# stdstu12/YUME

Hardware: NVIDIA H100
Metric: latent_frames_per_sec (higher is better)
Workload: dtype bf16

## Files before the change

### include/yume_b200.h

```cpp
#ifndef YUME_B200_H_
#define YUME_B200_H_

#ifdef __cplusplus
extern "C" {
#endif

#define YB_OK 0
#define YB_ERR_ARG (-1)
#define YB_ERR_SHAPE (-2)
#define YB_ERR_ALIGNMENT (-3)
#define YB_ERR_NO_DRIVER (-4)
#define YB_ERR_TENSORMAP (-5)
#define YB_ERR_LAUNCH (-6)

int yb_abi_version(void);

#define YB_EPI_BF16 0
#define YB_EPI_GELU_BF16 1
#define YB_EPI_F32 2
#define YB_EPI_GATE_RES 3
#define YB_EPI_RES_BF16 5
#define YB_EPI_GELU_ERF_BF16 4

typedef struct yb_gemm_args {
// ... 3 lines not shown
  const void* B;
  const void* bias;
  void* out;
  const void* gate;
  const void* tok_idx;
  long long lda, ldb, ldo, gate_ld;
  int M, N, K;
  int epilogue;
  int block_n;
  int n_split;
  long long split_stride;
  int a_split;
  long long a_split_stride;
  const void* res;
  long long res_ld;
  int split_k;
  void* ws;
  long long ws_bytes;
} yb_gemm_args;
int yb_gemm_bf16(const yb_gemm_args* args, void* stream);
long long yb_gemm_workspace_bytes(int M, int N, int K, int epilogue, int cta_pair, int split_k);
int yb_gemm_splitk_plan(int tiles, int num_kb, int clusters, int split_k, int* out3);
int yb_gemm_plan(int M, int N, int sms, int* out4);

typedef struct yb_conv3d_args {
  unsigned int struct_bytes;
  int cta_pair;
  const void* xpad;
  const void* w;
  const void* bias;
  void* out;
  const void* res;
  long long ldo, res_ld;
  int T, H, W, Cp, Cout;
  int epilogue;
  int kt, kh, kw;
  int oob_zero_pad;
  int out_t_mul, out_t_add;
  int fuse_w;
  int stride_t, stride_hw;
} yb_conv3d_args;
int yb_conv3d_causal(const yb_conv3d_args* args, void* stream);
int yb_conv3d_plan(int T, int H, int W, int Cout, int kw, int fuse_w, int* out4);

int yb_ln_modulate(const void* x, long long ldx, void* out, long long ldo, int out_f32, const void* scale,
                   const void* shift, long long mod_ld, const void* tok_idx, const void* weight, const void* lnbias,
// ... 77 lines not shown
```

### yume_b200/_lib.py

```python
from __future__ import annotations

import ctypes as C
from pathlib import Path

_LIB_PATH = Path(__file__).resolve().parent / "csrc" / "libyume_b200.so"

YB_EPI_BF16, YB_EPI_GELU_BF16, YB_EPI_F32, YB_EPI_GATE_RES, YB_EPI_GELU_ERF_BF16, YB_EPI_RES_BF16 = 0, 1, 2, 3, 4, 5
YB_ATT_P_SMEM, YB_ATT_ACCUMULATE = 1, 2
ABI_VERSION = 4
YB_ATT_EMU_SHIFT, YB_ATT_SPLIT_SHIFT = 2, 4

_ERRORS = {
    -1: "YB_ERR_ARG (null pointer / bad enum / non-positive size)",
    -2: "YB_ERR_SHAPE (shape not supported by the kernel)",
    -3: "YB_ERR_ALIGNMENT (pointer or stride not 16-byte aligned)",
    -4: "YB_ERR_NO_DRIVER (cuTensorMapEncodeTiled unavailable: no CUDA driver)",
    -5: "YB_ERR_TENSORMAP (driver rejected a TMA descriptor)",
    -6: "YB_ERR_LAUNCH (kernel launch failed)",
}


class YumeB200Error(RuntimeError):
    pass

# ... 15 lines not shown
class Conv3dArgs(C.Structure):

    _fields_ = [
        ("struct_bytes", C.c_uint), ("cta_pair", C.c_int),
        ("xpad", C.c_void_p), ("w", C.c_void_p), ("bias", C.c_void_p), ("out", C.c_void_p), ("res", C.c_void_p),
        ("ldo", C.c_longlong), ("res_ld", C.c_longlong),
        ("T", C.c_int), ("H", C.c_int), ("W", C.c_int), ("Cp", C.c_int), ("Cout", C.c_int), ("epilogue", C.c_int),
        ("kt", C.c_int), ("kh", C.c_int), ("kw", C.c_int), ("oob_zero_pad", C.c_int), ("out_t_mul", C.c_int),
        ("out_t_add", C.c_int), ("fuse_w", C.c_int), ("stride_t", C.c_int), ("stride_hw", C.c_int),
    ]


_vp, _ll, _i, _f = C.c_void_p, C.c_longlong, C.c_int, C.c_float
SIGNATURES = {
    "yb_abi_version": (_i, []),
    "yb_gemm_bf16": (_i, [C.POINTER(GemmArgs), _vp]),
    "yb_conv3d_causal": (_i, [C.POINTER(Conv3dArgs), _vp]),
    "yb_gn_stats": (_i, [_vp, _ll, _vp, _ll, _i, _i, _vp]),
    "yb_vae_pad_act": (_i, [_vp, _ll, _i, _i, _i, _i, _vp, _i, _i, _i, _i, _i, _vp, _vp, _vp, _i, _f, _i, _vp]),
    "yb_masked_softmax": (_i, [_vp, _ll, _vp, _ll, _i, _i, _vp]),
    "yb_nchw_to_nhwc_bf16": (_i, [_vp, _vp, _ll, _i, _i, _vp]),
    "yb_nhwc_to_nchw_f32": (_i, [_vp, _ll, _vp, _ll, _i, _vp]),
    "yb_gemm_plan": (_i, [_i, _i, _i, C.POINTER(C.c_int)]),
    "yb_gemm_workspace_bytes": (_ll, [_i, _i, _i, _i, _i, _i]),
    "yb_gemm_splitk_plan": (_i, [_i, _i, _i, _i, C.POINTER(C.c_int)]),
    "yb_conv3d_plan": (_i, [_i, _i, _i, _i, _i, _i, C.POINTER(C.c_int)]),
    "yb_attention_plan": (_i, [_i, _i, _i, _i, _i, C.POINTER(C.c_int)]),
    "yb_nhwc_to_nchw_f32_clamp": (_i, [_vp, _ll, _vp, _ll, _i, C.c_float, C.c_float, _vp]),
    "yb_blend": (_i, [_vp, _vp, _ll, _i, _i, _i, _ll, _vp]),
    "yb_vae_assemble_tiles": (_i, [_vp, _vp, _vp, _vp, _vp, _i, _i, _i, _i, _i, _i, _i, _i, _i, _i, _i, _vp, _vp]),
    "yb_vae_rms_act": (_i, [_vp, _ll, _vp, _vp, _i, _i, _i, _i, _i, _i, _i, _vp]),
    "yb_vae_dupup_add": (_i, [_vp, _vp, _i, _i, _i, _i, _i, _i, _i, _vp]),
    "yb_vae_unpatchify2_clamp": (_i, [_vp, _ll, _vp, _i, _i, _i, _vp]),
    "yb_vae_avgdown_add": (_i, [_vp, _vp, _i, _i, _i, _i, _i, _i, _i, _vp]),
    "yb_vae_patchify2_bf16": (_i, [_vp, _vp, _ll, _i, _i, _i, _vp]),
    "yb_ln_modulate": (_i, [_vp, _ll, _vp, _ll, _i, _vp, _vp, _ll, _vp, _vp, _vp, _i, _i, _f, _vp]),
    "yb_rmsnorm_rope": (_i, [_vp, _ll, _vp, _vp, _i, _i, _i, _i, _f, _vp]),
    "yb_rmsnorm_rope_pieces": (_i, [_vp, _ll, _i, _ll, _vp, _vp, _i, _i, _i, _i, _f, _vp]),
    "yb_qk_norm_rope": (_i, [_vp, _vp, _ll, _i, _ll, _vp, _vp, _vp, _i, _i, _i, _i, _f, _vp]),
    "yb_attention": (_i, [_vp, _ll, _vp, _ll, _vp, _ll, _vp, _ll, _i, _i, _i, _f, _i, _vp]),
    "yb_attention_ex": (_i, [_vp, _ll, _vp, _ll, _vp, _ll, _vp, _ll, _i, _i, _i, _f, _i, _vp, _ll, _vp, _vp]),
    "yb_attention_workspace_bytes": (_ll, [_i, _i, _i, _i, _i]),
    "yb_debug_force_split": (_i, [_i]),
    "yb_sp_scatter_qkv": (_i, [_vp, _ll, _vp, _vp, _vp, _i, _i, _i, _i, _f, C.POINTER(C.c_void_p), _i, _i, _i, _vp]),
    "yb_gemm_sp_qkv": (_i, [_vp, _ll, _vp, _vp, _i, _i, _i, C.POINTER(C.c_void_p), _i, _i, _i, _vp, _vp]),
    "yb_sp_bcast_sums": (_i, [_vp, C.POINTER(C.c_void_p), _i, _i, _i, _vp]),
# ... 107 lines not shown
```

### yume_b200/csrc/gemm.cu

```cuda
#include "yb_host.h"
#include "../../include/yume_b200_stream.h"
#include "yb_ptx.cuh"

namespace yb {

constexpr int GEMM_BLOCK_M = 128;
constexpr int GEMM_BLOCK_K = 64;
constexpr int GEMM_THREADS = 384;
constexpr int GEMM_MAX_STAGES = 8;
constexpr int GEMM_SMEM_BYTES = 227 * 1024;
constexpr int GEMM_A_BYTES = GEMM_BLOCK_M * GEMM_BLOCK_K * 2;
constexpr int GEMM_EPI_STAGE_BYTES = 8 * 16 * 36 * 4;
constexpr int GEMM_EPI_BOX_BYTES = 64 * 128;
constexpr int GEMM_EPI_TMA_BYTES = 2 * 2 * GEMM_EPI_BOX_BYTES;

struct GemmParams {
  int M, N, K;
  const float* bias;
  void* out;
  long long ldo;
  const float* gate;
  long long gate_ld;
  const int* tok_idx;
  int a_split;
// ... 6 lines not shown
  int cT, cH, cW;
  int kh, kw;
  int off_t, off_h, off_w;
  int out_t_mul, out_t_add;
  int st_t, st_h, st_w;
  int num_m_tiles, num_n_tiles;
  int block_n, stages;
  int sk_full, sk_ns, sk_per;
  float* sk_ws;
  int tma_out;
  __nv_bfloat16* sp_peers[8];
  float* sp_sums;
  int sp_rank, sp_Lp, sp_Wh, sp_C;
};
constexpr int YB_EPI_SP_QKV = 6;

constexpr int CONVW_ROWS = GEMM_BLOCK_M + 2;
constexpr int CONVW_A_SLAB = 17 * 1024;
constexpr int CONVW_A_STAGES = 4;

__host__ __device__ constexpr int gemm_b_bytes(int block_n) { return ((block_n + 63) / 64) * 64 * GEMM_BLOCK_K * 2; }
__host__ __device__ constexpr int gemm_stage_bytes(int block_n, int convw) { return (convw ? 0 : GEMM_A_BYTES) + gemm_b_bytes(block_n); }
__host__ __device__ constexpr int gemm_a_ring_bytes(int convw) { return convw ? CONVW_A_STAGES * CONVW_A_SLAB : 0; }
__host__ __device__ constexpr bool gemm_has_tma_epilogue(int epi, int convw, int cluster) {
  return cluster == 1 && !convw && (epi == YB_EPI_BF16 || epi == YB_EPI_GELU_BF16 || epi == YB_EPI_GELU_ERF_BF16 ||
                                    epi == YB_EPI_F32 || epi == YB_EPI_GATE_RES);
}
__host__ __device__ constexpr bool gemm_tma_epilogue_only(int epi, int convw, int cluster) {
  return gemm_has_tma_epilogue(epi, convw, cluster) && epi != YB_EPI_BF16 && epi != YB_EPI_F32;
}
__host__ __device__ constexpr int gemm_epi_bytes(bool tma) { return tma ? GEMM_EPI_TMA_BYTES : GEMM_EPI_STAGE_BYTES; }
static int gemm_stages(int block_n, int convw, int epi_bytes) {
  const int s = (GEMM_SMEM_BYTES - 1024 - 256 - epi_bytes - gemm_a_ring_bytes(convw)) / gemm_stage_bytes(block_n, convw);
  return s > GEMM_MAX_STAGES ? GEMM_MAX_STAGES : s;
}

template <int EPI>
__device__ __forceinline__ void epilogue_rows16(const GemmParams& p, int col0, int my_row, int my_tok, const float* stage, int lane,
                                                float* sq) {
  constexpr bool kBf16Out = (EPI == YB_EPI_BF16 || EPI == YB_EPI_GELU_BF16 || EPI == YB_EPI_GELU_ERF_BF16 ||
                             EPI == YB_EPI_RES_BF16 || EPI == YB_EPI_SP_QKV);
  if (col0 >= p.N) return;
  if (kBf16Out) {
    const int cq = (lane & 3) * 8;
    float b[8] = {0.f, 0.f, 0.f, 0.f, 0.f, 0.f, 0.f, 0.f};
    if (p.bias) {
      const float4 b0 = __ldg(reinterpret_cast<const float4*>(p.bias + col0 + cq));
      const float4 b1 = __ldg(reinterpret_cast<const float4*>(p.bias + col0 + cq + 4));
      b[0] = b0.x; b[1] = b0.y; b[2] = b0.z; b[3] = b0.w; b[4] = b1.x; b[5] = b1.y; b[6] = b1.z; b[7] = b1.w;
    }
    long long col_off = col0 + cq;
    if (p.n_split > 0) col_off = static_cast<long long>(col0 / p.n_split) * p.split_stride + (col0 % p.n_split) + cq;
// ... 170 lines not shown
}

template <int NM>
__device__ __forceinline__ void gemm_mma_k64(float (&acc)[128], uint32_t sa, uint32_t sb, int block_n, bool zero_first) {
  const uint64_t ad0 = make_smem_desc_sw128(sa, 16, 1024), bd0 = make_smem_desc_sw128(sb, 16, 1024);
  const int nb64 = (block_n + 63) >> 6;
#pragma unroll
  for (int k = 0; k < GEMM_BLOCK_K / 16; ++k) {
    const uint64_t ad = ad0 + 2 * k, bd = bd0 + 2 * k;
    const uint32_t accum = (zero_first && k == 0) ? 0u : 1u;
    if (NM == 256) {
      wgmma_ss_n256<0>(acc, ad, bd, accum);
    } else if (NM == 128) {
      wgmma_ss_n128<0>(acc, ad, bd, accum);
    } else {
      wgmma_ss_n64<0>(acc, ad, bd, accum);
      if (nb64 > 1) wgmma_ss_n64<32>(acc, ad, bd + (8192 >> 4), accum);
      if (nb64 > 2) wgmma_ss_n64<64>(acc, ad, bd + (16384 >> 4), accum);
      if (nb64 > 3) wgmma_ss_n64<96>(acc, ad, bd + (24576 >> 4), accum);
    }
  }
}

template <int CLUSTER>
__device__ __forceinline__ void release_slot(uint64_t* bar, int lane) {
  __syncwarp();
  if (lane == 0) {
    if (CLUSTER == 1) {
      mbar_arrive(bar);
    } else {
      mbar_arrive_cluster(bar, 0);
      mbar_arrive_cluster(bar, 1);
    }
  }
}

template <int EPI, int CONVW, int CLUSTER, int NM>
__global__ void __launch_bounds__(GEMM_THREADS, 1)
gemm_kernel(const __grid_constant__ CUtensorMap tmA, const __grid_constant__ CUtensorMap tmB, const __grid_constant__ CUtensorMap tmO,
            const GemmParams p) {
  static_assert(!(CONVW && CLUSTER != 1), "the kw-fused conv runs on single CTAs");
  constexpr bool kTmaEpi = gemm_has_tma_epilogue(EPI, CONVW, CLUSTER);
  const bool tma_out = gemm_tma_epilogue_only(EPI, CONVW, CLUSTER) || (kTmaEpi && p.tma_out);
  extern __shared__ uint8_t smem_raw[];
  uint8_t* smem = reinterpret_cast<uint8_t*>((reinterpret_cast<uintptr_t>(smem_raw) + 1023) & ~uintptr_t(1023));
  const int block_n = p.block_n, stages = p.stages;
  const int stage_bytes = gemm_stage_bytes(block_n, CONVW);
  uint8_t* a_ring = smem + stages * stage_bytes;
  float* epi = reinterpret_cast<float*>(a_ring + gemm_a_ring_bytes(CONVW));
  uint64_t* full_bar = reinterpret_cast<uint64_t*>(reinterpret_cast<uint8_t*>(epi) + gemm_epi_bytes(kTmaEpi));
  uint64_t* empty_bar = full_bar + GEMM_MAX_STAGES;
  uint64_t* a_full = empty_bar + GEMM_MAX_STAGES;
  uint64_t* a_empty = a_full + CONVW_A_STAGES;

  const int warp = threadIdx.x >> 5, lane = threadIdx.x & 31;
  const int rank = CLUSTER == 2 ? static_cast<int>(cluster_ctarank()) : 0;
  const int tile_first = blockIdx.x / CLUSTER, tile_step = gridDim.x / CLUSTER;
  const int num_tiles = p.num_m_tiles * p.num_n_tiles;
  const int num_kb = (p.K + GEMM_BLOCK_K - 1) / GEMM_BLOCK_K;
  const int num_work = p.sk_full + (num_tiles - p.sk_full) * p.sk_ns;
  auto decode_work = [&](int w, int& tile, int& kb0, int& kb1, int& part) {
    tile = w; kb0 = 0; kb1 = num_kb; part = -1;
    if (w >= p.sk_full) {
      const int u = w - p.sk_full;
      tile = p.sk_full + u / p.sk_ns;
      kb0 = (u % p.sk_ns) * p.sk_per;
      kb1 = min(num_kb, kb0 + p.sk_per);
      part = u;
    }
  };
  auto conv_box = [&](int mt, int& it, int& ih, int& iw) {
    const int per_t = p.tiles_h * p.tiles_w;
    it = mt / per_t;
    const int rem = mt - it * per_t;
    ih = rem / p.tiles_w;
    iw = rem - ih * p.tiles_w;
  };

  if (threadIdx.x == 0) {
    tma_prefetch_desc(&tmA);
    tma_prefetch_desc(&tmB);
    if (tma_out) tma_prefetch_desc(&tmO);
    for (int i = 0; i < stages; ++i) {
      mbar_init(&full_bar[i], 1);
      mbar_init(&empty_bar[i], 8 * CLUSTER);
    }
    for (int i = 0; i < (CONVW ? CONVW_A_STAGES : 0); ++i) {
      mbar_init(&a_full[i], 1);
      mbar_init(&a_empty[i], 8);
    }
    fence_barrier_init();
  }
  __syncthreads();
  if (CLUSTER > 1) cluster_sync_all();

  if (warp < 4) {
    setmaxnreg_dec<40>();
    if (warp == 0 && lane == 0) {
      int stage = 0, a_stage = 0;
      uint32_t phase = 0, a_phase = 0;
      for (int w = tile_first; w < num_work; w += tile_step) {
        int tile, kb0, kb1, part, m_tile, n_tile;
        decode_work(w, tile, kb0, kb1, part);
        tile_coords(tile, p.num_m_tiles, p.num_n_tiles, m_tile, n_tile);
        if (CONVW) {
          int it, ih, iw;
          conv_box(m_tile, it, ih, iw);
          const int groups = num_kb / 3;
// ... 3 lines not shown
            mbar_wait(&a_empty[a_stage], a_phase ^ 1);
            mbar_arrive_expect_tx(&a_full[a_stage], CONVW_ROWS * GEMM_BLOCK_K * 2);
            tma_load_4d(a_ring + a_stage * CONVW_A_SLAB, &tmA, &a_full[a_stage], cc * GEMM_BLOCK_K, iw * GEMM_BLOCK_M - p.off_w,
                        ih + dh - p.off_h, it + dt - p.off_t);
            if (++a_stage == CONVW_A_STAGES) {
              a_stage = 0;
              a_phase ^= 1;
            }
#pragma unroll 1
            for (int dw = 0; dw < 3; ++dw) {
              mbar_wait(&empty_bar[stage], phase ^ 1);
              mbar_arrive_expect_tx(&full_bar[stage], block_n * GEMM_BLOCK_K * 2);
              tma_load_2d(smem + stage * stage_bytes, &tmB, &full_bar[stage], ((tdh * 3 + dw) * p.cin_chunks + cc) * GEMM_BLOCK_K,
                          n_tile * block_n);
              if (++stage == stages) {
                stage = 0;
                phase ^= 1;
              }
            }
          }
          continue;
        }
        for (int kb = kb0; kb < kb1; ++kb) {
          if (CLUSTER > 1) mbar_wait_cluster(&empty_bar[stage], phase ^ 1);
          else mbar_wait(&empty_bar[stage], phase ^ 1);
          uint8_t* sa = smem + stage * stage_bytes;
          uint8_t* sb = sa + GEMM_A_BYTES;
          mbar_arrive_expect_tx(&full_bar[stage], GEMM_A_BYTES + block_n * GEMM_BLOCK_K * 2);
          const int kcol = kb * GEMM_BLOCK_K;
          const int mt = m_tile * CLUSTER + rank;
          if (p.conv) {
            const int tap = kb / p.cin_chunks, cc = kb - tap * p.cin_chunks;
            const int dt = tap / (p.kh * p.kw), dh = (tap / p.kw) % p.kh, dw = tap % p.kw;
            int it, ih, iw;
            conv_box(mt, it, ih, iw);
            tma_load_4d(sa, &tmA, &full_bar[stage], cc * GEMM_BLOCK_K, iw * p.TW * p.st_w + dw - p.off_w,
                        ih * p.TH * p.st_h + dh - p.off_h, it * p.TT * p.st_t + dt - p.off_t);
          } else {
            const int chunk = kcol / p.a_split;
            tma_load_3d(sa, &tmA, &full_bar[stage], kcol - chunk * p.a_split, mt * GEMM_BLOCK_M, chunk);
          }
          if (CLUSTER == 1) {
            tma_load_2d(sb, &tmB, &full_bar[stage], kcol, n_tile * block_n);
          } else {
            const int half = block_n / 2;
            tma_load_2d_multicast(sb + rank * half * GEMM_BLOCK_K * 2, &tmB, &full_bar[stage], kcol, n_tile * block_n + rank * half,
                                  static_cast<uint16_t>(3));
          }
          if (++stage == stages) {
            stage = 0;
            phase ^= 1;
          }
        }
      }
    }
  } else {
    setmaxnreg_inc<232>();
    const int wg = (warp >> 2) - 1;
    const int r0 = wg * 64 + (warp & 3) * 16;
    float* stage_buf = epi + (warp - 4) * (16 * 36);
    uint8_t* box_bufs = reinterpret_cast<uint8_t*>(epi) + wg * 2 * GEMM_EPI_BOX_BYTES;
    uint32_t nbox = 0;
    int stage = 0, a_stage = 0;
    uint32_t phase = 0, a_phase = 0;
    float acc[128];
// ... 20 lines not shown
      }
      if (EPI == YB_EPI_GATE_RES && part < 0 && my_row >= 0 && lane < 16) {
        const char* xrow = reinterpret_cast<const char*>(reinterpret_cast<const float*>(p.out) +
                                                         static_cast<long long>(my_row) * p.ldo + n_tile * block_n);
        const int ncols = min(block_n, p.N - n_tile * block_n);
        for (int b = 0; b < ncols * 4; b += 128) asm volatile("prefetch.global.L2 [%0];" ::"l"(xrow + b));
      }
      int prev = -1;
      if (CONVW) {
        int prev_a = -1;
        const int groups = num_kb / 3;
        for (int g = 0; g < groups; ++g) {
          mbar_wait(&a_full[a_stage], a_phase);
          const uint32_t sa = smem_u32(a_ring + a_stage * CONVW_A_SLAB) + wg * 64 * 128;
#pragma unroll 1
          for (int dw = 0; dw < 3; ++dw) {
            mbar_wait(&full_bar[stage], phase);
            fence_regs(acc);
            wgmma_fence();
            gemm_mma_k64<NM>(acc, sa + dw * 128, smem_u32(smem + stage * stage_bytes), block_n, g == 0 && dw == 0);
            wgmma_commit();
            wgmma_wait<1>();
            fence_regs(acc);
            if (prev >= 0) release_slot<1>(&empty_bar[prev], lane);
            if (dw == 0 && prev_a >= 0) {
              release_slot<1>(&a_empty[prev_a], lane);
              prev_a = -1;
            }
            prev = stage;
            if (++stage == stages) {
              stage = 0;
              phase ^= 1;
            }
          }
          prev_a = a_stage;
          if (++a_stage == CONVW_A_STAGES) {
            a_stage = 0;
            a_phase ^= 1;
          }
        }
        wgmma_wait<0>();
        fence_regs(acc);
        if (prev >= 0) release_slot<1>(&empty_bar[prev], lane);
        if (prev_a >= 0) release_slot<1>(&a_empty[prev_a], lane);
      } else {
        for (int kb = kb0; kb < kb1; ++kb) {
          mbar_wait(&full_bar[stage], phase);
          const uint32_t sa = smem_u32(smem + stage * stage_bytes);
          fence_regs(acc);
          wgmma_fence();
          gemm_mma_k64<NM>(acc, sa + wg * 64 * 128, sa + GEMM_A_BYTES, block_n, kb == kb0);
          wgmma_commit();
          wgmma_wait<1>();
          fence_regs(acc);
          if (prev >= 0) release_slot<CLUSTER>(&empty_bar[prev], lane);
          prev = stage;
          if (++stage == stages) {
            stage = 0;
            phase ^= 1;
          }
        }
        wgmma_wait<0>();
        fence_regs(acc);
        if (prev >= 0) release_slot<CLUSTER>(&empty_bar[prev], lane);
      }

      const int q4 = lane >> 2, c2 = 2 * (lane & 3);
      if (part >= 0) {
        float* wbase = p.sk_ws + (static_cast<long long>(part) * 256 + rank * GEMM_BLOCK_M + r0) * block_n;
#pragma unroll
        for (int g = 0; g < 32; ++g) {
          if (g * 8 < block_n) {
            *reinterpret_cast<float2*>(wbase + q4 * block_n + g * 8 + c2) = make_float2(acc[4 * g], acc[4 * g + 1]);
            *reinterpret_cast<float2*>(wbase + (q4 + 8) * block_n + g * 8 + c2) = make_float2(acc[4 * g + 2], acc[4 * g + 3]);
          }
        }
        continue;
      }
      if (tma_out) {
        epilogue_tma<EPI, NM>(p, &tmO, acc, box_bufs, mt * GEMM_BLOCK_M + wg * 64, n_tile * block_n, wg, threadIdx.x & 127, nbox);
        continue;
      }
      int my_tok = 0;
      if (EPI == YB_EPI_GATE_RES && p.gate != nullptr && p.tok_idx != nullptr && my_row >= 0) my_tok = p.tok_idx[my_row];
      float sq[2] = {0.f, 0.f};
      auto flush_sq = [&](int part_) {
#pragma unroll
// ... 101 lines not shown
}

template <typename Kern>
static int pair_max_clusters(Kern kern) {
  cudaLaunchConfig_t cfg = {};
  cfg.gridDim = dim3(2 * (sm_count() / 2));
  cfg.blockDim = dim3(GEMM_THREADS);
  cfg.dynamicSmemBytes = GEMM_SMEM_BYTES;
  cudaLaunchAttribute attr;
  attr.id = cudaLaunchAttributeClusterDimension;
  attr.val.clusterDim.x = 2;
  attr.val.clusterDim.y = 1;
  attr.val.clusterDim.z = 1;
  cfg.attrs = &attr;
  cfg.numAttrs = 1;
  int n = 0;
  if (cudaOccupancyMaxActiveClusters(&n, kern, &cfg) != cudaSuccess || n <= 0) {
    (void)cudaGetLastError();
    n = sm_count() / 2;
  }
  return n;
}

template <int EPI, int CONVW, int CLUSTER>
static int launch_gemm(const CUtensorMap& tmA, const CUtensorMap& tmB, const CUtensorMap* tmO, GemmParams& p, cudaStream_t stream,
                       int split_k = 1, void* ws = nullptr, long long ws_bytes = 0) {
  static const CUtensorMap no_map = {};
  if (gemm_tma_epilogue_only(EPI, CONVW, CLUSTER) && tmO == nullptr) return YB_ERR_ARG;
  p.tma_out = gemm_has_tma_epilogue(EPI, CONVW, CLUSTER) && tmO != nullptr;
  if (!p.tma_out) tmO = &no_map;
  const int nm = p.block_n == 256 ? 2 : p.block_n == 128 ? 1 : 0;
  if (CLUSTER == 1 && nm == 0) return YB_ERR_ARG;
  auto kern = nm == 2 ? gemm_kernel<EPI, CONVW, CLUSTER, 256> : nm == 1 ? gemm_kernel<EPI, CONVW, CLUSTER, 128>
                      : gemm_kernel<EPI, CONVW, CLUSTER, CLUSTER == 1 ? 128 : 64>;
  static bool attr_set[3][kMaxDevices] = {};
  if (int rc = ensure_dynamic_smem(kern, GEMM_SMEM_BYTES, attr_set[nm], "gemm")) return rc;
  if (CLUSTER == 2) p.num_m_tiles = p.conv ? (p.num_m_tiles + 1) / 2 : (p.M + 255) / 256;
  else if (!p.conv) p.num_m_tiles = (p.M + GEMM_BLOCK_M - 1) / GEMM_BLOCK_M;
  p.num_n_tiles = (p.N + p.block_n - 1) / p.block_n;
  p.stages = gemm_stages(p.block_n, CONVW, gemm_epi_bytes(gemm_has_tma_epilogue(EPI, CONVW, CLUSTER)));
  const int tiles = p.num_m_tiles * p.num_n_tiles;
  static int max_clusters[kMaxDevices] = {0};
  const int dev = current_device();
  if (max_clusters[dev] == 0) max_clusters[dev] = CLUSTER == 2 ? pair_max_clusters(kern) : sm_count();
  p.sk_full = tiles; p.sk_ns = 1; p.sk_per = 0; p.sk_ws = nullptr;
  int tail = 0;
  if (CLUSTER == 2 && EPI == YB_EPI_GATE_RES && !p.conv && ws != nullptr && split_k != 1) {
    const int num_kb = (p.K + GEMM_BLOCK_K - 1) / GEMM_BLOCK_K;
    gemm_splitk_plan(tiles, num_kb, max_clusters[dev], split_k, &p.sk_full, &p.sk_ns, &p.sk_per);
    tail = tiles - p.sk_full;
    const long long need = static_cast<long long>(tail) * p.sk_ns * 256 * p.block_n * 4;
    if (tail > 0 && (ws_bytes < need || (reinterpret_cast<uintptr_t>(ws) & 0xF))) {
      p.sk_full = tiles; p.sk_ns = 1; tail = 0;
    }
    if (tail > 0) p.sk_ws = static_cast<float*>(ws);
  }
  const int work = p.sk_full + tail * p.sk_ns;
  const int groups = work < max_clusters[dev] ? work : max_clusters[dev];
  cudaLaunchConfig_t cfg = {};
  cfg.gridDim = dim3(groups * CLUSTER);
  cfg.blockDim = dim3(GEMM_THREADS);
  cfg.dynamicSmemBytes = GEMM_SMEM_BYTES;
  cfg.stream = stream;
// ... 85 lines not shown
  if (tiles <= 0 || num_kb <= 0 || clusters <= 0 || split_k < 0 || split_k > 12 || !out3) return YB_ERR_ARG;
  yb::gemm_splitk_plan(tiles, num_kb, clusters, split_k, &out3[0], &out3[1], &out3[2]);
  return YB_OK;
}

extern "C" long long yb_gemm_workspace_bytes(int M, int N, int K, int epilogue, int cta_pair, int split_k) {
  using namespace yb;
  if (M <= 0 || N <= 0 || K <= 0 || epilogue != YB_EPI_GATE_RES || split_k == 1 || split_k < 0 || split_k > 12) return 0;
  if (cta_pair != 2) return 0;
  static int max_clusters[kMaxDevices] = {0};
  static bool attr_set[kMaxDevices] = {false};
  const int dev = current_device();
  if (max_clusters[dev] == 0) {
    if (ensure_dynamic_smem(gemm_kernel<YB_EPI_GATE_RES, 0, 2, 256>, GEMM_SMEM_BYTES, attr_set, "gemm")) return 0;
    max_clusters[dev] = pair_max_clusters(gemm_kernel<YB_EPI_GATE_RES, 0, 2, 256>);
  }
  const int bn = pair_block_n(M, N, max_clusters[dev]);
  const int tiles = ((M + 255) / 256) * ((N + bn - 1) / bn);
  int full, ns, per;
  gemm_splitk_plan(tiles, (K + GEMM_BLOCK_K - 1) / GEMM_BLOCK_K, max_clusters[dev], split_k, &full, &ns, &per);
  return static_cast<long long>(tiles - full) * ns * 256 * bn * 4;
}

extern "C" int yb_gemm_bf16(const yb_gemm_args* a, void* stream_) {
  using namespace yb;
  if (!a || !a->A || !a->B || !a->out) return YB_ERR_ARG;
  if (a->M <= 0 || a->N <= 0 || a->K <= 0) return YB_ERR_ARG;
  if (a->N % 32 != 0 || a->K % 8 != 0) return YB_ERR_SHAPE;
  if (a->epilogue < 0 || a->epilogue > YB_EPI_RES_BF16) return YB_ERR_ARG;
  if (a->epilogue == YB_EPI_RES_BF16 && (!a->res || (a->res_ld % 8))) return YB_ERR_ARG;
  if ((a->lda % 8) || (a->ldb % 8) || (a->ldo % 8) || (reinterpret_cast<uintptr_t>(a->out) & 0xF)) return YB_ERR_ALIGNMENT;
  cudaStream_t stream = reinterpret_cast<cudaStream_t>(stream_);
  if (a->struct_bytes != sizeof(yb_gemm_args)) return YB_ERR_ARG;
  if (a->cta_pair < 0 || a->cta_pair > 2 || a->split_k < 0 || a->split_k > 12) return YB_ERR_ARG;
  int a_split = a->K;
  long long a_chunk_ld = 0;
  if (a->a_split > 0) {
    if (a->a_split % GEMM_BLOCK_K != 0 || a->K % a->a_split != 0) return YB_ERR_SHAPE;
    a_split = a->a_split;
    a_chunk_ld = a->a_split_stride;
  }
  const int a_chunks = a->K / a_split;
  if (a->n_split < 0 || (a->n_split > 0 && (a->n_split % 32 != 0 || a->epilogue != YB_EPI_BF16))) return YB_ERR_ARG;
  GemmParams p;
  p.M = a->M;
  p.N = a->N;
  p.K = a->K;
  p.bias = static_cast<const float*>(a->bias);
  p.out = a->out;
  p.ldo = a->ldo;
  p.gate = static_cast<const float*>(a->gate);
  p.gate_ld = a->gate_ld;
  p.tok_idx = static_cast<const int*>(a->tok_idx);
  p.a_split = a_split;
  p.res = static_cast<const __nv_bfloat16*>(a->res);
  p.res_ld = a->res_ld;
  p.conv = 0;
// ... 3 lines not shown
  p.stages = 0;
  CUtensorMap tmA, tmB;
  int rc = make_tmap_bf16_3d(&tmA, a->A, a_chunks, a->M, a_split, a->lda, a_chunks > 1 ? a_chunk_ld : a->lda * (long long)a->M + 8,
                             GEMM_BLOCK_M, GEMM_BLOCK_K);
  if (rc) return rc;
  const bool pair = a->cta_pair == 2;
  if (pair) {
    int bn = a->block_n;
    if (bn == 0) bn = pair_block_n(a->M, a->N, sm_count() / 2);
    if (bn < 32 || bn > 256 || bn % 32 != 0) return YB_ERR_ARG;
    p.block_n = bn;
    rc = make_tmap_bf16_2d(&tmB, a->B, a->N, a->K, a->ldb, bn / 2, GEMM_BLOCK_K);
    if (rc) return rc;
    switch (a->epilogue) {
      case YB_EPI_BF16: return launch_gemm<YB_EPI_BF16, 0, 2>(tmA, tmB, nullptr, p, stream);
      case YB_EPI_GELU_BF16: return launch_gemm<YB_EPI_GELU_BF16, 0, 2>(tmA, tmB, nullptr, p, stream);
      case YB_EPI_F32: return launch_gemm<YB_EPI_F32, 0, 2>(tmA, tmB, nullptr, p, stream);
      case YB_EPI_GELU_ERF_BF16: return launch_gemm<YB_EPI_GELU_ERF_BF16, 0, 2>(tmA, tmB, nullptr, p, stream);
      case YB_EPI_RES_BF16: return launch_gemm<YB_EPI_RES_BF16, 0, 2>(tmA, tmB, nullptr, p, stream);
      default: return launch_gemm<YB_EPI_GATE_RES, 0, 2>(tmA, tmB, nullptr, p, stream, a->split_k, a->ws, a->ws_bytes);
    }
  }
  const int block_n = (a->block_n == 128 || a->block_n == 256) ? a->block_n : ((a->N % 256 == 0 || a->N > 1024) ? 256 : 128);
  rc = make_tmap_bf16_2d(&tmB, a->B, a->N, a->K, a->ldb, block_n, GEMM_BLOCK_K);
  if (rc) return rc;
  p.block_n = block_n;
  CUtensorMap tmO;
  const CUtensorMap* tmo = nullptr;
  if (a->n_split == 0 && a->epilogue != YB_EPI_RES_BF16) {
    const int elem = (a->epilogue == YB_EPI_F32 || a->epilogue == YB_EPI_GATE_RES) ? 4 : 2;
    rc = make_tmap_out_2d(&tmO, a->out, a->M, a->N, a->ldo, elem, 64);
    if (rc) return rc;
    tmo = &tmO;
  }
  switch (a->epilogue) {
    case YB_EPI_BF16: return launch_gemm<YB_EPI_BF16, 0, 1>(tmA, tmB, tmo, p, stream);
    case YB_EPI_GELU_BF16: return launch_gemm<YB_EPI_GELU_BF16, 0, 1>(tmA, tmB, tmo, p, stream);
    case YB_EPI_F32: return launch_gemm<YB_EPI_F32, 0, 1>(tmA, tmB, tmo, p, stream);
    case YB_EPI_GELU_ERF_BF16: return launch_gemm<YB_EPI_GELU_ERF_BF16, 0, 1>(tmA, tmB, tmo, p, stream);
    case YB_EPI_RES_BF16: return launch_gemm<YB_EPI_RES_BF16, 0, 1>(tmA, tmB, nullptr, p, stream);
    default: return launch_gemm<YB_EPI_GATE_RES, 0, 1>(tmA, tmB, tmo, p, stream);
  }
}


static int conv3d_launch(const yb_conv3d_args* a, int t_hist, void* stream_) {
  using namespace yb;
  if (!a || !a->xpad || !a->w || !a->out) return YB_ERR_ARG;
  if (a->struct_bytes != sizeof(yb_conv3d_args)) return YB_ERR_ARG;
  if (a->T <= 0 || a->H <= 0 || a->W <= 0 || a->Cp <= 0 || a->Cout <= 0) return YB_ERR_ARG;
  if (t_hist < 0) return YB_ERR_ARG;
  if (a->Cp % 64 != 0 || a->Cout % 32 != 0) return YB_ERR_SHAPE;
  if ((a->ldo % 8) || (reinterpret_cast<uintptr_t>(a->out) & 0xF)) return YB_ERR_ALIGNMENT;
  if (a->epilogue != YB_EPI_BF16 && a->epilogue != YB_EPI_F32 && a->epilogue != YB_EPI_RES_BF16) return YB_ERR_ARG;
  if (a->epilogue == YB_EPI_RES_BF16 && (!a->res || (a->res_ld % 8))) return YB_ERR_ARG;
  cudaStream_t stream = reinterpret_cast<cudaStream_t>(stream_);
  GemmParams p;
  const int kt = a->kt > 0 ? a->kt : 3, kh = a->kh > 0 ? a->kh : 3, kw = a->kw > 0 ? a->kw : 3;
  if ((kt != 1 && kt != 3) || (kh != 1 && kh != 3) || (kw != 1 && kw != 3)) return YB_ERR_SHAPE;
  const int block_n = (a->Cout % 256 == 0) ? 256 : 128;
  bool fuse_w = false;
  if (a->cta_pair < 0 || a->cta_pair > 2) return YB_ERR_ARG;
  const int st_t = a->stride_t > 0 ? a->stride_t : 1, st_hw = a->stride_hw > 0 ? a->stride_hw : 1;
  if (st_t > 2 || st_hw > 2) return YB_ERR_ARG;
  const bool strided = st_t > 1 || st_hw > 1;
  if (strided && !a->oob_zero_pad) return YB_ERR_ARG;
  if (t_hist > 0 && (!a->oob_zero_pad || t_hist != (st_t > 1 ? 1 : kt - 1))) return YB_ERR_ARG;
// ... 75 lines not shown
```

### yume_b200/csrc/yb_ptx.cuh

```cuda
#pragma once
#include <cstdint>
#include <cstdio>
#include <cuda.h>
#include <cuda_runtime.h>
#include <cuda_bf16.h>

namespace yb {

__device__ __forceinline__ uint32_t smem_u32(const void* p) {
  return static_cast<uint32_t>(__cvta_generic_to_shared(p));
}

template <int N>
__device__ __forceinline__ void setmaxnreg_inc() {
  asm volatile("setmaxnreg.inc.sync.aligned.u32 %0;\n" ::"n"(N));
}
template <int N>
__device__ __forceinline__ void setmaxnreg_dec() {
  asm volatile("setmaxnreg.dec.sync.aligned.u32 %0;\n" ::"n"(N));
}
__device__ __forceinline__ void named_bar_sync(int id, int count) {
  asm volatile("bar.sync %0, %1;" ::"r"(id), "r"(count) : "memory");
}

// ... 69 lines not shown
  const long long t0 = clock64();
  for (;;) {
    uint32_t ok;
    asm volatile(
        "{\n\t.reg .pred p;\n\t"
        "mbarrier.try_wait.parity.acquire.cluster.shared::cta.b64 p, [%1], %2;\n\t"
        "selp.u32 %0, 1, 0, p;\n\t}\n"
        : "=r"(ok)
        : "r"(smem_u32(bar)), "r"(parity)
        : "memory");
    if (ok) return;
    if (clock64() - t0 > YB_WAIT_LIMIT_CYCLES) __trap();
  }
}

__device__ __forceinline__ uint32_t cluster_ctarank() {
  uint32_t r;
  asm volatile("mov.u32 %0, %%cluster_ctarank;" : "=r"(r));
  return r;
}
__device__ __forceinline__ void cluster_sync_all() {
  asm volatile("barrier.cluster.arrive.release.aligned;\n\tbarrier.cluster.wait.acquire.aligned;" ::: "memory");
}
__device__ __forceinline__ void mbar_arrive_cluster(uint64_t* bar, uint32_t cta) {
  uint32_t remote;
  asm volatile("mapa.shared::cluster.u32 %0, %1, %2;" : "=r"(remote) : "r"(smem_u32(bar)), "r"(cta));
  asm volatile("mbarrier.arrive.release.cluster.shared::cluster.b64 _, [%0];" ::"r"(remote) : "memory");
}

__device__ __forceinline__ void tma_prefetch_desc(const CUtensorMap* tmap) {
  asm volatile("prefetch.tensormap [%0];" ::"l"(reinterpret_cast<uint64_t>(tmap)) : "memory");
}
__device__ __forceinline__ void tma_load_2d(void* smem_dst, const CUtensorMap* tmap, uint64_t* bar, int c0, int c1) {
  asm volatile(
      "cp.async.bulk.tensor.2d.shared::cluster.global.tile.mbarrier::complete_tx::bytes [%0], [%1, {%3, %4}], [%2];"
      ::"r"(smem_u32(smem_dst)), "l"(reinterpret_cast<uint64_t>(tmap)), "r"(smem_u32(bar)), "r"(c0), "r"(c1)
      : "memory");
}
__device__ __forceinline__ void tma_load_2d_multicast(void* smem_dst, const CUtensorMap* tmap, uint64_t* bar, int c0, int c1,
                                                      uint16_t mask) {
  asm volatile(
      "cp.async.bulk.tensor.2d.shared::cluster.global.mbarrier::complete_tx::bytes.multicast::cluster [%0], [%1, {%3, %4}], "
      "[%2], %5;" ::"r"(smem_u32(smem_dst)),
      "l"(reinterpret_cast<uint64_t>(tmap)), "r"(smem_u32(bar)), "r"(c0), "r"(c1), "h"(mask)
      : "memory");
}
// ... 150 lines not shown
```

Measured before the change: 42.12.

## Route large plain GEMMs to CTA-pair kernel with multicast B and TMA epilogue

Adds a CTA-pair (cluster of 2) GEMM path for large plain-epilogue GEMMs (M≥16384, N divisible by 256, large N*K). The pair multicasts half-width B tiles to both CTAs, uses a TMA store epilogue, and disables the split-K tail. By default the empty-slot release now uses CTA-scope remote arrives with a local wait instead of cluster-scope ones. This targets the B operand bandwidth and per-CTA load traffic of the big transformer linears, at the cost of cross-CTA synchronization and losing split-K balancing on the tail. Probe variants are compiled only under a macro.

```diff
diff --git a/include/yume_b200.h b/include/yume_b200.h
--- a/include/yume_b200.h
+++ b/include/yume_b200.h
@@ -49,6 +49,7 @@
 long long yb_gemm_workspace_bytes(int M, int N, int K, int epilogue, int cta_pair, int split_k);
 int yb_gemm_splitk_plan(int tiles, int num_kb, int clusters, int split_k, int* out3);
 int yb_gemm_plan(int M, int N, int sms, int* out4);
+int yb_gemm_pair_plan(int M, int N, int K, int epilogue);
 
 typedef struct yb_conv3d_args {
   unsigned int struct_bytes;
diff --git a/yume_b200/_lib.py b/yume_b200/_lib.py
--- a/yume_b200/_lib.py
+++ b/yume_b200/_lib.py
@@ -61,6 +61,7 @@
     "yb_nchw_to_nhwc_bf16": (_i, [_vp, _vp, _ll, _i, _i, _vp]),
     "yb_nhwc_to_nchw_f32": (_i, [_vp, _ll, _vp, _ll, _i, _vp]),
     "yb_gemm_plan": (_i, [_i, _i, _i, C.POINTER(C.c_int)]),
+    "yb_gemm_pair_plan": (_i, [_i, _i, _i, _i]),
     "yb_gemm_workspace_bytes": (_ll, [_i, _i, _i, _i, _i, _i]),
     "yb_gemm_splitk_plan": (_i, [_i, _i, _i, _i, C.POINTER(C.c_int)]),
     "yb_conv3d_plan": (_i, [_i, _i, _i, _i, _i, _i, C.POINTER(C.c_int)]),
diff --git a/yume_b200/csrc/gemm.cu b/yume_b200/csrc/gemm.cu
--- a/yume_b200/csrc/gemm.cu
+++ b/yume_b200/csrc/gemm.cu
@@ -52,12 +52,17 @@
 __host__ __device__ constexpr int gemm_b_bytes(int block_n) { return ((block_n + 63) / 64) * 64 * GEMM_BLOCK_K * 2; }
 __host__ __device__ constexpr int gemm_stage_bytes(int block_n, int convw) { return (convw ? 0 : GEMM_A_BYTES) + gemm_b_bytes(block_n); }
 __host__ __device__ constexpr int gemm_a_ring_bytes(int convw) { return convw ? CONVW_A_STAGES * CONVW_A_SLAB : 0; }
-__host__ __device__ constexpr bool gemm_has_tma_epilogue(int epi, int convw, int cluster) {
-  return cluster == 1 && !convw && (epi == YB_EPI_BF16 || epi == YB_EPI_GELU_BF16 || epi == YB_EPI_GELU_ERF_BF16 ||
-                                    epi == YB_EPI_F32 || epi == YB_EPI_GATE_RES);
-}
-__host__ __device__ constexpr bool gemm_tma_epilogue_only(int epi, int convw, int cluster) {
-  return gemm_has_tma_epilogue(epi, convw, cluster) && epi != YB_EPI_BF16 && epi != YB_EPI_F32;
+constexpr int PAIR_TMA_EPI = 8;
+constexpr int PROBE_OWN_B = 1;
+constexpr int PROBE_LOCAL_RELEASE = 2;
+constexpr int PROBE_CLUSTER_SCOPE = 4;
+
+__host__ __device__ constexpr bool gemm_has_tma_epilogue(int epi, int convw, int cluster, int form) {
+  return (cluster == 1 || (form & PAIR_TMA_EPI)) && !convw &&
+         (epi == YB_EPI_BF16 || epi == YB_EPI_GELU_BF16 || epi == YB_EPI_GELU_ERF_BF16 || epi == YB_EPI_F32 || epi == YB_EPI_GATE_RES);
+}
+__host__ __device__ constexpr bool gemm_tma_epilogue_only(int epi, int convw, int cluster, int form) {
+  return gemm_has_tma_epilogue(epi, convw, cluster, form) && (cluster == 2 || (epi != YB_EPI_BF16 && epi != YB_EPI_F32));
 }
 __host__ __device__ constexpr int gemm_epi_bytes(bool tma) { return tma ? GEMM_EPI_TMA_BYTES : GEMM_EPI_STAGE_BYTES; }
 static int gemm_stages(int block_n, int convw, int epi_bytes) {
@@ -274,26 +279,33 @@
   }
 }
 
-template <int CLUSTER>
+template <int CLUSTER, int FORM>
 __device__ __forceinline__ void release_slot(uint64_t* bar, int lane) {
   __syncwarp();
   if (lane == 0) {
-    if (CLUSTER == 1) {
+    if (CLUSTER == 1 || (FORM & PROBE_LOCAL_RELEASE)) {
       mbar_arrive(bar);
-    } else {
+    } else if (FORM & PROBE_CLUSTER_SCOPE) {
       mbar_arrive_cluster(bar, 0);
       mbar_arrive_cluster(bar, 1);
-    }
-  }
-}
-
-template <int EPI, int CONVW, int CLUSTER, int NM>
+    } else {
+      mbar_arrive_remote(bar, 0);
+      mbar_arrive_remote(bar, 1);
+    }
+  }
+}
+
+template <int EPI, int CONVW, int CLUSTER, int NM, int FORM = 0>
 __global__ void __launch_bounds__(GEMM_THREADS, 1)
 gemm_kernel(const __grid_constant__ CUtensorMap tmA, const __grid_constant__ CUtensorMap tmB, const __grid_constant__ CUtensorMap tmO,
             const GemmParams p) {
   static_assert(!(CONVW && CLUSTER != 1), "the kw-fused conv runs on single CTAs");
-  constexpr bool kTmaEpi = gemm_has_tma_epilogue(EPI, CONVW, CLUSTER);
-  const bool tma_out = gemm_tma_epilogue_only(EPI, CONVW, CLUSTER) || (kTmaEpi && p.tma_out);
+  static_assert(!(FORM & PAIR_TMA_EPI) || (CLUSTER == 2 && NM == 256), "the pair's TMA form runs 256-wide tiles");
+  constexpr bool kTmaEpi = gemm_has_tma_epilogue(EPI, CONVW, CLUSTER, FORM);
+  constexpr bool kMulticast = CLUSTER == 2 && !(FORM & PROBE_OWN_B);
+  constexpr int kReleasers = (CLUSTER == 2 && !(FORM & PROBE_LOCAL_RELEASE)) ? 2 : 1;
+  constexpr bool kSplitTail = !(FORM & PAIR_TMA_EPI);
+  const bool tma_out = gemm_tma_epilogue_only(EPI, CONVW, CLUSTER, FORM) || (kTmaEpi && p.tma_out);
   extern __shared__ uint8_t smem_raw[];
   uint8_t* smem = reinterpret_cast<uint8_t*>((reinterpret_cast<uintptr_t>(smem_raw) + 1023) & ~uintptr_t(1023));
   const int block_n = p.block_n, stages = p.stages;
@@ -313,7 +325,7 @@
   const int num_work = p.sk_full + (num_tiles - p.sk_full) * p.sk_ns;
   auto decode_work = [&](int w, int& tile, int& kb0, int& kb1, int& part) {
     tile = w; kb0 = 0; kb1 = num_kb; part = -1;
-    if (w >= p.sk_full) {
+    if (kSplitTail && w >= p.sk_full) {
       const int u = w - p.sk_full;
       tile = p.sk_full + u / p.sk_ns;
       kb0 = (u % p.sk_ns) * p.sk_per;
@@ -335,7 +347,7 @@
     if (tma_out) tma_prefetch_desc(&tmO);
     for (int i = 0; i < stages; ++i) {
       mbar_init(&full_bar[i], 1);
-      mbar_init(&empty_bar[i], 8 * CLUSTER);
+      mbar_init(&empty_bar[i], 8 * kReleasers);
     }
     for (int i = 0; i < (CONVW ? CONVW_A_STAGES : 0); ++i) {
       mbar_init(&a_full[i], 1);
@@ -385,7 +397,7 @@
           continue;
         }
         for (int kb = kb0; kb < kb1; ++kb) {
-          if (CLUSTER > 1) mbar_wait_cluster(&empty_bar[stage], phase ^ 1);
+          if (FORM & PROBE_CLUSTER_SCOPE) mbar_wait_cluster(&empty_bar[stage], phase ^ 1);
           else mbar_wait(&empty_bar[stage], phase ^ 1);
           uint8_t* sa = smem + stage * stage_bytes;
           uint8_t* sb = sa + GEMM_A_BYTES;
@@ -403,7 +415,7 @@
             const int chunk = kcol / p.a_split;
             tma_load_3d(sa, &tmA, &full_bar[stage], kcol - chunk * p.a_split, mt * GEMM_BLOCK_M, chunk);
           }
-          if (CLUSTER == 1) {
+          if (!kMulticast) {
             tma_load_2d(sb, &tmB, &full_bar[stage], kcol, n_tile * block_n);
           } else {
             const int half = block_n / 2;
@@ -470,9 +482,9 @@
             wgmma_commit();
             wgmma_wait<1>();
             fence_regs(acc);
-            if (prev >= 0) release_slot<1>(&empty_bar[prev], lane);
+            if (prev >= 0) release_slot<1, 0>(&empty_bar[prev], lane);
             if (dw == 0 && prev_a >= 0) {
-              release_slot<1>(&a_empty[prev_a], lane);
+              release_slot<1, 0>(&a_empty[prev_a], lane);
               prev_a = -1;
             }
             prev = stage;
@@ -489,8 +501,8 @@
         }
         wgmma_wait<0>();
         fence_regs(acc);
-        if (prev >= 0) release_slot<1>(&empty_bar[prev], lane);
-        if (prev_a >= 0) release_slot<1>(&a_empty[prev_a], lane);
+        if (prev >= 0) release_slot<1, 0>(&empty_bar[prev], lane);
+        if (prev_a >= 0) release_slot<1, 0>(&a_empty[prev_a], lane);
       } else {
         for (int kb = kb0; kb < kb1; ++kb) {
           mbar_wait(&full_bar[stage], phase);
@@ -501,7 +513,7 @@
           wgmma_commit();
           wgmma_wait<1>();
           fence_regs(acc);
-          if (prev >= 0) release_slot<CLUSTER>(&empty_bar[prev], lane);
+          if (prev >= 0) release_slot<CLUSTER, FORM>(&empty_bar[prev], lane);
           prev = stage;
           if (++stage == stages) {
             stage = 0;
@@ -510,7 +522,7 @@
         }
         wgmma_wait<0>();
         fence_regs(acc);
-        if (prev >= 0) release_slot<CLUSTER>(&empty_bar[prev], lane);
+        if (prev >= 0) release_slot<CLUSTER, FORM>(&empty_bar[prev], lane);
       }
 
       const int q4 = lane >> 2, c2 = 2 * (lane & 3);
@@ -658,23 +670,28 @@
   return n;
 }
 
-template <int EPI, int CONVW, int CLUSTER>
+template <int EPI, int CONVW, int CLUSTER, int FORM = 0>
 static int launch_gemm(const CUtensorMap& tmA, const CUtensorMap& tmB, const CUtensorMap* tmO, GemmParams& p, cudaStream_t stream,
                        int split_k = 1, void* ws = nullptr, long long ws_bytes = 0) {
   static const CUtensorMap no_map = {};
-  if (gemm_tma_epilogue_only(EPI, CONVW, CLUSTER) && tmO == nullptr) return YB_ERR_ARG;
-  p.tma_out = gemm_has_tma_epilogue(EPI, CONVW, CLUSTER) && tmO != nullptr;
+  constexpr bool has_tma_epi = gemm_has_tma_epilogue(EPI, CONVW, CLUSTER, FORM);
+  if (gemm_tma_epilogue_only(EPI, CONVW, CLUSTER, FORM) && tmO == nullptr) return YB_ERR_ARG;
+  p.tma_out = has_tma_epi && tmO != nullptr;
   if (!p.tma_out) tmO = &no_map;
   const int nm = p.block_n == 256 ? 2 : p.block_n == 128 ? 1 : 0;
-  if (CLUSTER == 1 && nm == 0) return YB_ERR_ARG;
-  auto kern = nm == 2 ? gemm_kernel<EPI, CONVW, CLUSTER, 256> : nm == 1 ? gemm_kernel<EPI, CONVW, CLUSTER, 128>
-                      : gemm_kernel<EPI, CONVW, CLUSTER, CLUSTER == 1 ? 128 : 64>;
+  if ((CLUSTER == 1 && nm == 0) || (FORM != 0 && nm != 2)) return YB_ERR_ARG;
+  auto kern = gemm_kernel<EPI, CONVW, CLUSTER, 256, FORM>;
+  if constexpr (FORM == 0) {
+    if (nm == 1) kern = gemm_kernel<EPI, CONVW, CLUSTER, 128>;
+    if (nm == 0) kern = gemm_kernel<EPI, CONVW, CLUSTER, CLUSTER == 1 ? 128 : 64>;
+  }
   static bool attr_set[3][kMaxDevices] = {};
   if (int rc = ensure_dynamic_smem(kern, GEMM_SMEM_BYTES, attr_set[nm], "gemm")) return rc;
   if (CLUSTER == 2) p.num_m_tiles = p.conv ? (p.num_m_tiles + 1) / 2 : (p.M + 255) / 256;
   else if (!p.conv) p.num_m_tiles = (p.M + GEMM_BLOCK_M - 1) / GEMM_BLOCK_M;
   p.num_n_tiles = (p.N + p.block_n - 1) / p.block_n;
-  p.stages = gemm_stages(p.block_n, CONVW, gemm_epi_bytes(gemm_has_tma_epilogue(EPI, CONVW, CLUSTER)));
+  const int ring = gemm_stages(p.block_n, CONVW, gemm_epi_bytes(has_tma_epi));
+  p.stages = ((FORM & ~PAIR_TMA_EPI) != 0 && p.stages > 0 && p.stages < ring) ? p.stages : ring;
   const int tiles = p.num_m_tiles * p.num_n_tiles;
   static int max_clusters[kMaxDevices] = {0};
   const int dev = current_device();
@@ -806,6 +823,20 @@
   return static_cast<long long>(tiles - full) * ns * 256 * bn * 4;
 }
 
+namespace yb {
+constexpr int PAIR_MIN_M = 16384;
+constexpr long long PAIR_MIN_NK = 3072LL * 9216;
+static bool gemm_pair_plan(int M, int N, int K, int epilogue) {
+  const bool plain = epilogue == YB_EPI_BF16 || epilogue == YB_EPI_GELU_BF16 || epilogue == YB_EPI_F32 || epilogue == YB_EPI_GATE_RES;
+  return plain && N % 256 == 0 && M >= PAIR_MIN_M && static_cast<long long>(N) * K >= PAIR_MIN_NK;
+}
+}
+
+extern "C" int yb_gemm_pair_plan(int M, int N, int K, int epilogue) {
+  if (M <= 0 || N <= 0 || K <= 0) return YB_ERR_ARG;
+  return yb::gemm_pair_plan(M, N, K, epilogue) ? 1 : 0;
+}
+
 extern "C" int yb_gemm_bf16(const yb_gemm_args* a, void* stream_) {
   using namespace yb;
   if (!a || !a->A || !a->B || !a->out) return YB_ERR_ARG;
@@ -816,7 +847,7 @@
   if ((a->lda % 8) || (a->ldb % 8) || (a->ldo % 8) || (reinterpret_cast<uintptr_t>(a->out) & 0xF)) return YB_ERR_ALIGNMENT;
   cudaStream_t stream = reinterpret_cast<cudaStream_t>(stream_);
   if (a->struct_bytes != sizeof(yb_gemm_args)) return YB_ERR_ARG;
-  if (a->cta_pair < 0 || a->cta_pair > 2 || a->split_k < 0 || a->split_k > 12) return YB_ERR_ARG;
+  if (a->cta_pair < 0 || a->cta_pair > 3 || a->split_k < 0 || a->split_k > 12) return YB_ERR_ARG;
   int a_split = a->K;
   long long a_chunk_ld = 0;
   if (a->a_split > 0) {
@@ -866,8 +897,6 @@
     }
   }
   const int block_n = (a->block_n == 128 || a->block_n == 256) ? a->block_n : ((a->N % 256 == 0 || a->N > 1024) ? 256 : 128);
-  rc = make_tmap_bf16_2d(&tmB, a->B, a->N, a->K, a->ldb, block_n, GEMM_BLOCK_K);
-  if (rc) return rc;
   p.block_n = block_n;
   CUtensorMap tmO;
   const CUtensorMap* tmo = nullptr;
@@ -877,6 +906,20 @@
     if (rc) return rc;
     tmo = &tmO;
   }
+  const bool plain = tmo != nullptr && a->epilogue != YB_EPI_GELU_ERF_BF16 && block_n == 256;
+  if (a->cta_pair == 3 && !plain) return YB_ERR_ARG;
+  if (a->cta_pair == 3 || (a->cta_pair == 0 && plain && gemm_pair_plan(a->M, a->N, a->K, a->epilogue))) {
+    rc = make_tmap_bf16_2d(&tmB, a->B, a->N, a->K, a->ldb, block_n / 2, GEMM_BLOCK_K);
+    if (rc) return rc;
+    switch (a->epilogue) {
+      case YB_EPI_BF16: return launch_gemm<YB_EPI_BF16, 0, 2, PAIR_TMA_EPI>(tmA, tmB, tmo, p, stream);
+      case YB_EPI_GELU_BF16: return launch_gemm<YB_EPI_GELU_BF16, 0, 2, PAIR_TMA_EPI>(tmA, tmB, tmo, p, stream);
+      case YB_EPI_F32: return launch_gemm<YB_EPI_F32, 0, 2, PAIR_TMA_EPI>(tmA, tmB, tmo, p, stream);
+      default: return launch_gemm<YB_EPI_GATE_RES, 0, 2, PAIR_TMA_EPI>(tmA, tmB, tmo, p, stream);
+    }
+  }
+  rc = make_tmap_bf16_2d(&tmB, a->B, a->N, a->K, a->ldb, block_n, GEMM_BLOCK_K);
+  if (rc) return rc;
   switch (a->epilogue) {
     case YB_EPI_BF16: return launch_gemm<YB_EPI_BF16, 0, 1>(tmA, tmB, tmo, p, stream);
     case YB_EPI_GELU_BF16: return launch_gemm<YB_EPI_GELU_BF16, 0, 1>(tmA, tmB, tmo, p, stream);
@@ -887,6 +930,45 @@
   }
 }
 
+
+#ifdef YB_GEMM_PAIR_PROBE
+extern "C" int yb_gemm_pair_probe(const yb_gemm_args* a, int rung, int* info3, void* stream_) {
+  using namespace yb;
+  if (!a || !info3 || a->epilogue != YB_EPI_BF16 || a->N % 256 != 0 || a->K % 8 != 0 || rung < 0 || rung > 7) return YB_ERR_ARG;
+  cudaStream_t stream = reinterpret_cast<cudaStream_t>(stream_);
+  GemmParams p = {};
+  p.M = a->M; p.N = a->N; p.K = a->K;
+  p.bias = static_cast<const float*>(a->bias);
+  p.out = a->out;
+  p.ldo = a->ldo;
+  p.a_split = a->K;
+  p.block_n = 256;
+  p.stages = rung == 3 ? 3 : 0;
+  CUtensorMap tmA, tmB, tmO;
+  int rc = make_tmap_bf16_3d(&tmA, a->A, 1, a->M, a->K, a->lda, a->lda * (long long)a->M + 8, GEMM_BLOCK_M, GEMM_BLOCK_K);
+  if (rc) return rc;
+  const bool own_b = rung == 0 || rung == 1 || rung == 5;
+  rc = make_tmap_bf16_2d(&tmB, a->B, a->N, a->K, a->ldb, own_b ? 256 : 128, GEMM_BLOCK_K);
+  if (rc) return rc;
+  rc = make_tmap_out_2d(&tmO, a->out, a->M, a->N, a->ldo, 2, 64);
+  if (rc) return rc;
+  static bool attr_set[kMaxDevices] = {};
+  if ((rc = ensure_dynamic_smem(gemm_kernel<YB_EPI_BF16, 0, 2, 256>, GEMM_SMEM_BYTES, attr_set, "gemm"))) return rc;
+  info3[0] = pair_max_clusters(gemm_kernel<YB_EPI_BF16, 0, 2, 256>);
+  switch (rung) {
+    case 0: rc = launch_gemm<YB_EPI_BF16, 0, 2, PROBE_OWN_B | PROBE_LOCAL_RELEASE>(tmA, tmB, nullptr, p, stream); break;
+    case 1: rc = launch_gemm<YB_EPI_BF16, 0, 2, PROBE_OWN_B | PROBE_CLUSTER_SCOPE>(tmA, tmB, nullptr, p, stream); break;
+    case 2: case 3: rc = launch_gemm<YB_EPI_BF16, 0, 2, PROBE_CLUSTER_SCOPE>(tmA, tmB, nullptr, p, stream); break;
+    case 4: rc = launch_gemm<YB_EPI_BF16, 0, 2, PROBE_CLUSTER_SCOPE | PAIR_TMA_EPI>(tmA, tmB, &tmO, p, stream); break;
+    case 5: rc = launch_gemm<YB_EPI_BF16, 0, 2, PROBE_OWN_B>(tmA, tmB, nullptr, p, stream); break;
+    case 6: rc = launch_gemm<YB_EPI_BF16, 0, 2>(tmA, tmB, nullptr, p, stream); break;
+    default: rc = launch_gemm<YB_EPI_BF16, 0, 2, PAIR_TMA_EPI>(tmA, tmB, &tmO, p, stream); break;
+  }
+  info3[1] = p.stages;
+  info3[2] = p.num_m_tiles * p.num_n_tiles;
+  return rc;
+}
+#endif
 
 static int conv3d_launch(const yb_conv3d_args* a, int t_hist, void* stream_) {
   using namespace yb;
diff --git a/yume_b200/csrc/yb_ptx.cuh b/yume_b200/csrc/yb_ptx.cuh
--- a/yume_b200/csrc/yb_ptx.cuh
+++ b/yume_b200/csrc/yb_ptx.cuh
@@ -115,6 +115,11 @@
 __device__ __forceinline__ void cluster_sync_all() {
   asm volatile("barrier.cluster.arrive.release.aligned;\n\tbarrier.cluster.wait.acquire.aligned;" ::: "memory");
 }
+__device__ __forceinline__ void mbar_arrive_remote(uint64_t* bar, uint32_t cta) {
+  uint32_t remote;
+  asm volatile("mapa.shared::cluster.u32 %0, %1, %2;" : "=r"(remote) : "r"(smem_u32(bar)), "r"(cta));
+  asm volatile("mbarrier.arrive.release.cta.shared::cluster.b64 _, [%0];" ::"r"(remote) : "memory");
+}
 __device__ __forceinline__ void mbar_arrive_cluster(uint64_t* bar, uint32_t cta) {
   uint32_t remote;
   asm volatile("mapa.shared::cluster.u32 %0, %1, %2;" : "=r"(remote) : "r"(smem_u32(bar)), "r"(cta));
```

New measurement: 42.48 (median of 6 runs). Within noise of the previous version (+0.9%).
